# leonzheng2/Safe-Exploration-with-Simulator-in-RL-algorithms

Hardware: AMD Instinct MI355X
Metric: env-steps/sec (higher is better)
Workload: dtype f64; 1 GPU; ARS V2 iteration, 3-segment swimmer, 512 directions/GPU x 2 rollouts x H=1000 (BASELINE configs[2] per GPU); directions_total=512, directions_per_gpu=512, horizon=1000, segments=3, trajectory_capture=True, full_covariance=True, parallelism=directions sharded over 1 GPU(s), 1 all-gather/iteration, ranks_seen=1

## Files before the change

include/swimmer_hip.h:

```cpp
#ifndef SWIMMER_HIP_H
#define SWIMMER_HIP_H

#include <stdint.h>

#ifdef __cplusplus
extern "C" {
#endif

#define SW_ABI_VERSION 3
#define SW_MAX_SEGMENTS 8

#define SW_OK 0
#define SW_ERR_NULL 1
#define SW_ERR_SEGMENTS 2
#define SW_ERR_SIZE 3
#define SW_ERR_PARAM 4
#define SW_ERR_LAUNCH 5

#define SW_STATUS_OK 0
#define SW_STATUS_SINGULAR 1
#define SW_STATUS_NONFINITE 2
#define SW_STATUS_RANGE 4
#define SW_STATUS_PARAM 8

#define SW_FLAG_ROLLOUT_LANE 1
#define SW_FLAG_ROLLOUT_QUAD 2

#define SW_FLAG_CAPTURE_SPLIT 8
#define SW_FLAG_CAPTURE_PACKED_V1 16
#define SW_FLAG_CAPTURE_LEAN_V1 128

#define SW_FLAG_MODEL_TWIN 4

typedef struct sw_params {
    int32_t n;
    int32_t flags;
    double l_i;
    double m_i;
    double k;
    double h;
    double dir_x;
    double dir_y;
} sw_params;

int sw_abi_version(void);
// ... 229 lines not shown
```

safe-exploration-with-simulator-in-rl-algorithms_amd/_build.py:

```python
import os
import shutil
import subprocess
import tempfile
from concurrent.futures import ThreadPoolExecutor

_HERE = os.path.dirname(os.path.abspath(__file__))
CSRC = os.path.join(_HERE, "csrc")
LIB_PATH = os.environ.get("SWIMMER_HIP_LIB") or os.path.join(CSRC, "libswimmer_hip.so")
OBJ_DIR = LIB_PATH + ".obj"
SOURCES = ["swimmer_kernels.hip", "swimmer_abi.hip", "swimmer_cacla.hip", "swimmer_lqr.hip", "swimmer_cacla_safe.hip",
           "swimmer_cacla_ensemble.hip", "swimmer_rlglue_ars.hip", "swimmer_safe_ars_ensemble.hip", "direct_comm.cpp",
           "host_rng.cpp"]
FAMILIES = ["swimmer_rollout_row.hip", "swimmer_rollout_n3.hip", "swimmer_rollout_lane.hip",
            "swimmer_rollout_safe_multi.hip", "swimmer_step.hip", "swimmer_cov.hip", "swimmer_update.hip"]
HOST_ONLY = {"host_rng.cpp"}
HEADERS = ["rlglue_env.cpp", os.path.join("..", "..", "include", "rlglue_swimmer.h"),
           "swimmer_launch.h", "swimmer_cov.h", "swimmer_device.h", "swimmer_rollout_lane.inc",
           "swimmer_rollout_quad3.inc", "swimmer_rollout_oct3.inc", "swimmer_rollout_octp3.inc",
           "swimmer_rollout_row.inc", "swimmer_rollout_multi.inc", "swimmer_rollout_safe_oct3.inc",
           "swimmer_rollout_safe_lane.inc", "swimmer_rollout_safe_multi.inc", "swimmer_update.inc", "swimmer_quad3.h",
           "swimmer_oct3.h", "swimmer_row.h", "swimmer_row_fused.h", "swimmer_twin.h", "swimmer_cacla_learner.h",
           "swimmer_cacla_gated.h", os.path.join("..", "..", "include", "swimmer_hip.h")] + FAMILIES
HIPCC_FLAGS = ["-O3", "--offload-arch=gfx950", "-std=c++17", "-fPIC"] + os.environ.get("SWIMMER_HIPCC_EXTRA", "").split()
HOST_FLAGS = ["-O3", "-std=c++17", "-fPIC"]
LINK_LIBS = ["-ldl"]
LLVM = "/opt/rocm/lib/llvm/bin"


def _hipcc():
    exe = shutil.which("hipcc") or "/opt/rocm/bin/hipcc"
    if not os.path.exists(exe):
        raise RuntimeError("hipcc not found: the swimmer HIP library cannot be built")
    return exe
# ... 79 lines not shown
```

safe-exploration-with-simulator-in-rl-algorithms_amd/_lib.py:

```python
import ctypes
import os

import numpy as np
import torch

from . import _build

ABI_VERSION = 3
MAX_SEGMENTS = 8

ERR_NAMES = {0: "SW_OK", 1: "SW_ERR_NULL", 2: "SW_ERR_SEGMENTS", 3: "SW_ERR_SIZE",
             4: "SW_ERR_PARAM", 5: "SW_ERR_LAUNCH"}
STATUS_SINGULAR = 1
STATUS_NONFINITE = 2
STATUS_RANGE = 4
STATUS_PARAM = 8
FLAG_ROLLOUT_LANE = 1
FLAG_ROLLOUT_QUAD = 2
FLAG_MODEL_TWIN = 4
FLAG_CAPTURE_SPLIT = 8
FLAG_CAPTURE_PACKED_V1 = 16
FLAG_CAPTURE_LEAN_V1 = 128
COST_ABS_OBS = 0
COST_MAX_ABS_THETADOT = 1


class SwParams(ctypes.Structure):
    _fields_ = [("n", ctypes.c_int32), ("flags", ctypes.c_int32), ("l_i", ctypes.c_double),
                ("m_i", ctypes.c_double), ("k", ctypes.c_double), ("h", ctypes.c_double),
                ("dir_x", ctypes.c_double), ("dir_y", ctypes.c_double)]

    @classmethod
    def make(cls, n=3, l_i=1.0, m_i=1.0, k=10.0, h=1e-3, direction=(1.0, 0.0), flags=0):
        return cls(int(n), int(flags), float(l_i), float(m_i), float(k), float(h),
                   float(direction[0]), float(direction[1]))

    @property
    def d(self):
        return 2 * self.n + 2

    @property
    def m(self):
        return self.n - 1


class SwimmerHipError(RuntimeError):
    pass


def kernel_flags(name):
    try:
        return {"auto": 0, "lane": FLAG_ROLLOUT_LANE, "quad": FLAG_ROLLOUT_QUAD, "split": FLAG_CAPTURE_SPLIT,
                "packed_v1": FLAG_CAPTURE_PACKED_V1, "lean_v1": FLAG_CAPTURE_LEAN_V1}[name]
    except KeyError:
        raise SwimmerHipError("rollout kernel must be 'auto', 'lane', 'quad', 'split', 'packed_v1' or 'lean_v1', "
                              f"not {name!r}")


_lib = None

_PROTOTYPES = {
    "sw_abi_version": (ctypes.c_int, []),
    "sw_max_segments": (ctypes.c_int, []),
    "sw_strerror": (ctypes.c_char_p, [ctypes.c_int]),
    "sw_moments_blocks": (ctypes.c_int64, [ctypes.c_int64]),
    "sw_reset_f64": (ctypes.c_int, [ctypes.c_void_p, ctypes.c_int64, ctypes.c_void_p,
                                    ctypes.c_void_p]),
    "sw_step_f64": (ctypes.c_int, [ctypes.c_void_p, ctypes.c_int64] + [ctypes.c_void_p] * 6),
    "sw_step_residual_f64": (ctypes.c_int, [ctypes.c_void_p, ctypes.c_int64] + [ctypes.c_void_p] * 5),
    "sw_step_residual_blocks": (ctypes.c_int64, [ctypes.c_int64]),
    "sw_step_residual_pop_f64": (ctypes.c_int, [ctypes.c_void_p, ctypes.c_int64, ctypes.c_void_p, ctypes.c_int64]
# ... 208 lines not shown
```

safe-exploration-with-simulator-in-rl-algorithms_amd/csrc/swimmer_launch.h:

```cpp
#pragma once
#include <hip/hip_runtime.h>
#include <math.h>
#include <stdint.h>
#include <climits>
#include <cstdlib>
#include <type_traits>
#include <utility>

#include "../../include/swimmer_hip.h"
#include "swimmer_device.h"
#include "swimmer_twin.h"

#define SW_PIN_LOOP(PAD) asm volatile(".p2align 6\n\t.fill %0, 4, 0xbf800000" ::"n"(PAD))
#ifndef SW_OCT_UNROLL
#define SW_OCT_UNROLL 8
#endif
#ifdef SW_OCT_LOOP_PAD
constexpr int oct_loop_pad(bool, bool) { return SW_OCT_LOOP_PAD; }
#else
constexpr int oct_loop_pad(bool traj, bool mom) { return traj ? (mom ? 5 : 6) : (mom ? 6 : 2); }
#endif
#ifndef SW_OCTP_LOOP_PAD
#define SW_OCTP_LOOP_PAD 4
#endif
constexpr int oct_packed_loop_pad() { return SW_OCTP_LOOP_PAD; }
#ifndef SW_OCTL_LOOP_PAD
#define SW_OCTL_LOOP_PAD 2
#endif
constexpr int oct_lean_loop_pad() { return SW_OCTL_LOOP_PAD; }
#ifndef SW_OCTS_LOOP_PAD
#define SW_OCTS_LOOP_PAD 2
#endif
constexpr int oct_next_e_loop_pad() { return SW_OCTS_LOOP_PAD; }
#ifndef SW_OCTS_TRIP16
#define SW_OCTS_TRIP16 1
#endif
#ifndef SW_QUAD_LOOP_PAD
#define SW_QUAD_LOOP_PAD 0
#endif
#ifdef SW_ROW_LOOP_PAD
constexpr int row_loop_pad(int, bool, bool) { return SW_ROW_LOOP_PAD; }
#else
constexpr int row_loop_pad(int n, bool traj, bool mom)
{
    if (n == 6 && !(traj && mom)) return traj ? 6 : 4;
    return n == 4 ? 5 : n == 5 ? 0 : n == 6 ? 5 : n == 7 ? 6 : 1;
}
#endif

#ifdef SW_MULTI_LOOP_PAD
// ... 77 lines not shown
    return sw::consts_of(p->n, p->l_i, p->m_i, p->k, p->h, p->dir_x, p->dir_y);
}

sw::TwinConsts make_twin_consts(const sw_params *p)
{
    return sw::TwinConsts{p->l_i, p->m_i, p->k, p->h, p->dir_x, p->dir_y};
}

inline bool is_twin(const sw_params *p) { return (p->flags & SW_FLAG_MODEL_TWIN) != 0; }

int validate_params(const sw_params *p)
{
    if (!p) return SW_ERR_NULL;
    if (p->n < 2 || p->n > SW_MAX_SEGMENTS) return SW_ERR_SEGMENTS;
    if (p->flags & ~(SW_FLAG_ROLLOUT_LANE | SW_FLAG_ROLLOUT_QUAD | SW_FLAG_MODEL_TWIN | SW_FLAG_CAPTURE_SPLIT |
                     SW_FLAG_CAPTURE_PACKED_V1 | SW_FLAG_CAPTURE_LEAN_V1))
        return SW_ERR_PARAM;
    if ((p->flags & SW_FLAG_CAPTURE_SPLIT) && (p->flags & SW_FLAG_CAPTURE_PACKED_V1)) return SW_ERR_PARAM;
    if ((p->flags & SW_FLAG_CAPTURE_LEAN_V1) && (p->flags & (SW_FLAG_CAPTURE_SPLIT | SW_FLAG_CAPTURE_PACKED_V1)))
        return SW_ERR_PARAM;
    if (!(p->l_i > 0.0) || !(p->m_i > 0.0) || !isfinite(p->l_i) || !isfinite(p->m_i) ||
        !isfinite(p->k) || !isfinite(p->h) || !isfinite(p->dir_x) || !isfinite(p->dir_y))
        return SW_ERR_PARAM;
    return SW_OK;
}

int check_params(const sw_params *p)
{
    (void)hipGetLastError();
    return validate_params(p);
}

int launch_status()
{
// ... 263 lines not shown
```

safe-exploration-with-simulator-in-rl-algorithms_amd/csrc/swimmer_rollout_n3.hip:

```cpp
#include "swimmer_cov.h"
#include "swimmer_quad3.h"
#include "swimmer_oct3.h"

namespace {

template <bool ARS, bool TRAJ, bool MOM>
__global__ void __launch_bounds__(kRollBlock)
rollout_quad3_kernel(sw::Consts C, int64_t n_roll, int32_t H, const double *__restrict__ policies,
                     const double *__restrict__ deltas, int64_t dir_begin, double nu,
                     const double *__restrict__ mean, const double *__restrict__ inv_std,
                     const double *__restrict__ state0, double *__restrict__ returns,
                     double *__restrict__ traj, double *__restrict__ final_state,
                     double *__restrict__ moments, int32_t *__restrict__ status, SideJob side)
{
#define SW_GATE_BODY 0
#include "swimmer_rollout_quad3.inc"
#undef SW_GATE_BODY
}

__global__ void __launch_bounds__(kRollBlock)
ars_gate_quad3_kernel(sw::Consts C, int64_t n_roll, int32_t H, const double *__restrict__ policies,
                      const double *__restrict__ deltas, int64_t dir_begin, double nu,
                      const double *__restrict__ mean, const double *__restrict__ inv_std, double gate_thr,
                      int32_t *__restrict__ admit, double *__restrict__ returns, int32_t *__restrict__ status,
// ... 39 lines not shown
#include "swimmer_rollout_oct3.inc"
#undef SW_GATE_BODY
}

template <bool ARS>
__global__ void __launch_bounds__(kOctBlock)
rollout_octp3_kernel(sw::Consts C, int64_t n_roll, int32_t H, const double *__restrict__ policies,
                     const double *__restrict__ deltas, int64_t dir_begin, double nu,
                     const double *__restrict__ mean, const double *__restrict__ inv_std,
                     const double *__restrict__ state0, double *__restrict__ returns,
                     double *__restrict__ traj, double *__restrict__ final_state,
                     double *__restrict__ moments, int32_t *__restrict__ status, SideJob side)
{
#define SW_OCTP_LEAN 0
#define SW_OCTP_NEXT_E 0
#include "swimmer_rollout_octp3.inc"
#undef SW_OCTP_NEXT_E
#undef SW_OCTP_LEAN
}

template <bool ARS>
__global__ void __launch_bounds__(kOctBlock)
rollout_octl3_kernel(sw::Consts C, int64_t n_roll, int32_t H, const double *__restrict__ policies,
                     const double *__restrict__ deltas, int64_t dir_begin, double nu,
                     const double *__restrict__ mean, const double *__restrict__ inv_std,
                     const double *__restrict__ state0, double *__restrict__ returns,
                     double *__restrict__ traj, double *__restrict__ final_state,
                     double *__restrict__ moments, int32_t *__restrict__ status, SideJob side)
{
#define SW_OCTP_LEAN 1
#define SW_OCTP_NEXT_E 0
#include "swimmer_rollout_octp3.inc"
#undef SW_OCTP_NEXT_E
#undef SW_OCTP_LEAN
}

template <bool ARS>
__global__ void __launch_bounds__(kOctBlock)
rollout_octs3_kernel(sw::Consts C, int64_t n_roll, int32_t H, const double *__restrict__ policies,
                     const double *__restrict__ deltas, int64_t dir_begin, double nu,
                     const double *__restrict__ mean, const double *__restrict__ inv_std,
                     const double *__restrict__ state0, double *__restrict__ returns,
                     double *__restrict__ traj, double *__restrict__ final_state,
                     double *__restrict__ moments, int32_t *__restrict__ status, SideJob side)
{
#define SW_OCTP_LEAN 1
#define SW_OCTP_NEXT_E 1
#include "swimmer_rollout_octp3.inc"
#undef SW_OCTP_NEXT_E
#undef SW_OCTP_LEAN
}

#define SW_MULTI_N 3
template <bool MOM>
__global__ void __launch_bounds__(kRollBlock)
ars_multi_quad3_kernel(sw::Consts C, int64_t n_roll, int32_t H, sw_launch::MultiArgs all, double nu, SideJob side)
{
    constexpr bool ARS = true, TRAJ = false;
#include "swimmer_rollout_multi.inc"
#define SW_GATE_BODY 0
#include "swimmer_rollout_quad3.inc"
#undef SW_GATE_BODY
}
// ... 105 lines not shown
                         double sim_thresh, double real_thresh, double *__restrict__ returns,
                         double *__restrict__ traj, int32_t *__restrict__ first_refused,
                         int32_t *__restrict__ violations, int32_t *__restrict__ status)
{
#define SW_SAFE_MULTI 0
#include "swimmer_rollout_safe_oct3.inc"
#undef SW_SAFE_MULTI
}

using namespace sw_launch;

int launch_oct3(const sw_params *p, const RolloutPlan &plan, bool ars, int64_t n_roll, int32_t H, const RolloutArgs &a,
                hipStream_t stream, const SideWork *side)
{
    if (a.traj && a.moments && !(p->flags & SW_FLAG_CAPTURE_SPLIT)) {
        with_bools([&](auto ARS, auto V1, auto LEAN_V1) {
            if constexpr (V1.value)
                launch_segment_per_lane(rollout_octp3_kernel<ARS.value>, p, plan, n_roll, H, a, stream, side);
            else if constexpr (LEAN_V1.value)
                launch_segment_per_lane(rollout_octl3_kernel<ARS.value>, p, plan, n_roll, H, a, stream, side);
            else
                launch_segment_per_lane(rollout_octs3_kernel<ARS.value>, p, plan, n_roll, H, a, stream, side);
        }, ars, (p->flags & SW_FLAG_CAPTURE_PACKED_V1) != 0, (p->flags & SW_FLAG_CAPTURE_LEAN_V1) != 0);
        return launch_status();
    }
    with_bools([&](auto ARS, auto TRAJ, auto MOM) {
        launch_segment_per_lane(rollout_oct3_kernel<ARS.value, TRAJ.value, MOM.value>, p, plan, n_roll, H, a, stream,
                                side);
    }, ars, a.traj != nullptr, a.moments != nullptr);
    return launch_status();
}

int launch_quad3(const sw_params *p, const RolloutPlan &plan, bool ars, int64_t n_roll, int32_t H,
                 const RolloutArgs &a, hipStream_t stream, const SideWork *side)
{
    with_bools([&](auto ARS, auto TRAJ, auto MOM) {
        launch_segment_per_lane(rollout_quad3_kernel<ARS.value, TRAJ.value, MOM.value>, p, plan, n_roll, H, a, stream,
// ... 118 lines not shown
```

safe-exploration-with-simulator-in-rl-algorithms_amd/csrc/swimmer_rollout_octp3.inc:

```
#ifndef SW_OCTP_LEAN
#error "define SW_OCTP_LEAN as 0 or 1 before including swimmer_rollout_octp3.inc"
#endif
#ifndef SW_OCTP_NEXT_E
#error "define SW_OCTP_NEXT_E as 0 or 1 before including swimmer_rollout_octp3.inc"
#endif
#if SW_OCTP_NEXT_E && !SW_OCTP_LEAN
#error "SW_OCTP_NEXT_E is a variant of the lean mode"
#endif
    side_flag(side);
    if (blockIdx.x >= side.first_cov_block) {
        side_cov_tile<8, kOctBlock>(side);
        return;
    }
    __builtin_amdgcn_s_setprio(3);
    constexpr int D = 8, M = 2;
    const int tid = threadIdx.x, lane = tid & (kWave - 1), wave = tid / kWave;
    const int q = lane & 3;
    const int seg = (q == 3) ? 0 : q;
    const bool cosine = (lane & 8) != 0;
    const int64_t r_raw = (int64_t)blockIdx.x * kMomGroup + wave * 8 + (lane >> 4) * 2 + ((lane >> 2) & 1);
    const bool valid = r_raw < n_roll;
    const int64_t r = valid ? r_raw : n_roll - 1;
    const sw::OctLane O = sw::oct3_lane(C, seg, cosine);
    const int cth = 2 + 2 * seg, cthd = 3 + 2 * seg;
// ... 100 lines not shown
        Gx = sw::oct3_geometry(A);
        det = sw::oct3_dynamics(C, O, Gc, Pu, Pv, thd, w1, w2, tq);
#endif
        const double Z = sw::octp3_pack(__builtin_fma(A.kd, sw::kPio2Hi, A.r), thd, Pu, lane3);
        const double X = Z - shift;
        m1 += X;
        m2 = __builtin_fma(X, X, m2);
        store_cell(Z);
#if !SW_OCTP_LEAN
        soff += slab;
#endif
        w1 = sw::dpp_f64<sw::kDppNext1>(thd);
        w2 = sw::dpp_f64<sw::kDppNext2>(thd);
        Pv = sw::dpp_row_f64<sw::kDppRowRor8>(Pu);
    };
    int32_t t = 0;
#if SW_OCTP_NEXT_E
    SW_PIN_LOOP(oct_next_e_loop_pad());
#else
    SW_PIN_LOOP(SW_OCTP_LEAN ? oct_lean_loop_pad() : oct_packed_loop_pad());
#endif
#if SW_OCTP_NEXT_E && SW_OCTS_TRIP16
    for (; t + 16 <= H; t += 16) {
        SW_OCTP_STEP_AT(0);   one_step(G, Gn);
        SW_OCTP_STEP_AT(k1);  one_step(Gn, G);
        SW_OCTP_STEP_AT(k2);  one_step(G, Gn);
        SW_OCTP_STEP_AT(k3);  one_step(Gn, G);
        SW_OCTP_STEP_AT(k4);  one_step(G, Gn);
        SW_OCTP_STEP_AT(k5);  one_step(Gn, G);
        SW_OCTP_STEP_AT(k6);  one_step(G, Gn);
        SW_OCTP_STEP_AT(k7);  one_step(Gn, G);
        SW_OCTP_STEP_AT(k8);  one_step(G, Gn);
        SW_OCTP_STEP_AT(k9);  one_step(Gn, G);
        SW_OCTP_STEP_AT(k10); one_step(G, Gn);
        SW_OCTP_STEP_AT(k11); one_step(Gn, G);
        SW_OCTP_STEP_AT(k12); one_step(G, Gn);
        SW_OCTP_STEP_AT(k13); one_step(Gn, G);
        SW_OCTP_STEP_AT(k14); one_step(G, Gn);
        SW_OCTP_STEP_AT(k15); one_step(Gn, G);
        SW_OCTP_TRIP_END(bump16);
    }
#endif
    for (; t + 8 <= H; t += 8) {
        SW_OCTP_STEP_AT(0);  one_step(G, Gn);
        SW_OCTP_STEP_AT(k1); one_step(Gn, G);
        SW_OCTP_STEP_AT(k2); one_step(G, Gn);
        SW_OCTP_STEP_AT(k3); one_step(Gn, G);
        SW_OCTP_STEP_AT(k4); one_step(G, Gn);
        SW_OCTP_STEP_AT(k5); one_step(Gn, G);
        SW_OCTP_STEP_AT(k6); one_step(G, Gn);
        SW_OCTP_STEP_AT(k7); one_step(Gn, G);
        SW_OCTP_TRIP_END(bump8);
    }
    for (; t + 4 <= H; t += 4) {
        SW_OCTP_STEP_AT(0);  one_step(G, Gn);
        SW_OCTP_STEP_AT(k1); one_step(Gn, G);
        SW_OCTP_STEP_AT(k2); one_step(G, Gn);
        SW_OCTP_STEP_AT(k3); one_step(Gn, G);
        SW_OCTP_TRIP_END(bump4);
    }
    for (; t + 2 <= H; t += 2) {
        SW_OCTP_STEP_AT(0);  one_step(G, Gn);
        SW_OCTP_STEP_AT(k1); one_step(Gn, G);
        SW_OCTP_TRIP_END(bump2);
    }
    SW_OCTP_STEP_AT(0);
    if (t < H) one_step(G, Gn);
#undef SW_OCTP_STEP_AT
#undef SW_OCTP_TRIP_END
    if (H > 0) th = __builtin_fma(A.kd, sw::kPio2Hi, A.r);
    thmax = fmax(thmax, fabs(th));

    int code = ((det > 0.0) ? 0 : SW_STATUS_SINGULAR) |
               ((isfinite(th) && isfinite(thd) && isfinite(Pu) && isfinite(Pv)) ? 0 : SW_STATUS_NONFINITE) |
               ((thmax < sw::kAngleLimit) ? 0 : SW_STATUS_RANGE);
    code |= __builtin_amdgcn_mov_dpp(code, sw::kDppNext1, 0xf, 0xf, true) |
            __builtin_amdgcn_mov_dpp(code, sw::kDppNext2, 0xf, 0xf, true);
    code |= __builtin_amdgcn_mov_dpp(code, sw::kDppRowRor8, 0xf, 0xf, true);
    const double sg_other = sw::dpp_row_f64<sw::kDppRowRor8>(m1);
    if (valid && !cosine && lane3) {
        const double total = __builtin_fma(C.dirx, m1, C.diry * sg_other);
        returns[r] = (code & SW_STATUS_RANGE) ? __builtin_nan("") : total;
// ... 37 lines not shown
```

Before: 5.000 billion env-steps/s.

## Add hand-scheduled two-step fused rollout kernel as default trajectory-capture path

New measurement: 4.623 billion env-steps/s. 0.925x the previous value.

```diff
diff --git a/include/swimmer_hip.h b/include/swimmer_hip.h
--- a/include/swimmer_hip.h
+++ b/include/swimmer_hip.h
@@ -29,6 +29,7 @@
 #define SW_FLAG_CAPTURE_SPLIT 8
 #define SW_FLAG_CAPTURE_PACKED_V1 16
 #define SW_FLAG_CAPTURE_LEAN_V1 128
+#define SW_FLAG_CAPTURE_NEXT_E_V1 512
 
 #define SW_FLAG_MODEL_TWIN 4
 
diff --git a/safe-exploration-with-simulator-in-rl-algorithms_amd/_build.py b/safe-exploration-with-simulator-in-rl-algorithms_amd/_build.py
--- a/safe-exploration-with-simulator-in-rl-algorithms_amd/_build.py
+++ b/safe-exploration-with-simulator-in-rl-algorithms_amd/_build.py
@@ -16,7 +16,7 @@
 HOST_ONLY = {"host_rng.cpp"}
 HEADERS = ["rlglue_env.cpp", os.path.join("..", "..", "include", "rlglue_swimmer.h"),
            "swimmer_launch.h", "swimmer_cov.h", "swimmer_device.h", "swimmer_rollout_lane.inc",
-           "swimmer_rollout_quad3.inc", "swimmer_rollout_oct3.inc", "swimmer_rollout_octp3.inc",
+           "swimmer_rollout_quad3.inc", "swimmer_rollout_oct3.inc", "swimmer_rollout_octp3.inc", "swimmer_rollout_octf3_pair.inc",
            "swimmer_rollout_row.inc", "swimmer_rollout_multi.inc", "swimmer_rollout_safe_oct3.inc",
            "swimmer_rollout_safe_lane.inc", "swimmer_rollout_safe_multi.inc", "swimmer_update.inc", "swimmer_quad3.h",
            "swimmer_oct3.h", "swimmer_row.h", "swimmer_row_fused.h", "swimmer_twin.h", "swimmer_cacla_learner.h",
diff --git a/safe-exploration-with-simulator-in-rl-algorithms_amd/_lib.py b/safe-exploration-with-simulator-in-rl-algorithms_amd/_lib.py
--- a/safe-exploration-with-simulator-in-rl-algorithms_amd/_lib.py
+++ b/safe-exploration-with-simulator-in-rl-algorithms_amd/_lib.py
@@ -21,6 +21,7 @@
 FLAG_CAPTURE_SPLIT = 8
 FLAG_CAPTURE_PACKED_V1 = 16
 FLAG_CAPTURE_LEAN_V1 = 128
+FLAG_CAPTURE_NEXT_E_V1 = 512
 COST_ABS_OBS = 0
 COST_MAX_ABS_THETADOT = 1
 
@@ -51,10 +52,11 @@
 def kernel_flags(name):
     try:
         return {"auto": 0, "lane": FLAG_ROLLOUT_LANE, "quad": FLAG_ROLLOUT_QUAD, "split": FLAG_CAPTURE_SPLIT,
-                "packed_v1": FLAG_CAPTURE_PACKED_V1, "lean_v1": FLAG_CAPTURE_LEAN_V1}[name]
+                "packed_v1": FLAG_CAPTURE_PACKED_V1, "lean_v1": FLAG_CAPTURE_LEAN_V1,
+                "next_e_v1": FLAG_CAPTURE_NEXT_E_V1}[name]
     except KeyError:
-        raise SwimmerHipError("rollout kernel must be 'auto', 'lane', 'quad', 'split', 'packed_v1' or 'lean_v1', "
-                              f"not {name!r}")
+        raise SwimmerHipError("rollout kernel must be 'auto', 'lane', 'quad', 'split', 'packed_v1', 'lean_v1' or "
+                              f"'next_e_v1', not {name!r}")
 
 
 _lib = None
diff --git a/safe-exploration-with-simulator-in-rl-algorithms_amd/csrc/swimmer_launch.h b/safe-exploration-with-simulator-in-rl-algorithms_amd/csrc/swimmer_launch.h
--- a/safe-exploration-with-simulator-in-rl-algorithms_amd/csrc/swimmer_launch.h
+++ b/safe-exploration-with-simulator-in-rl-algorithms_amd/csrc/swimmer_launch.h
@@ -34,6 +34,13 @@
 constexpr int oct_next_e_loop_pad() { return SW_OCTS_LOOP_PAD; }
 #ifndef SW_OCTS_TRIP16
 #define SW_OCTS_TRIP16 1
+#endif
+#ifndef SW_OCTF_LOOP_PAD
+#define SW_OCTF_LOOP_PAD 2
+#endif
+constexpr int oct_layout_loop_pad() { return SW_OCTF_LOOP_PAD; }
+#ifndef SW_OCTF_PROMOTE
+#define SW_OCTF_PROMOTE 0
 #endif
 #ifndef SW_QUAD_LOOP_PAD
 #define SW_QUAD_LOOP_PAD 0
@@ -141,10 +148,13 @@
     if (!p) return SW_ERR_NULL;
     if (p->n < 2 || p->n > SW_MAX_SEGMENTS) return SW_ERR_SEGMENTS;
     if (p->flags & ~(SW_FLAG_ROLLOUT_LANE | SW_FLAG_ROLLOUT_QUAD | SW_FLAG_MODEL_TWIN | SW_FLAG_CAPTURE_SPLIT |
-                     SW_FLAG_CAPTURE_PACKED_V1 | SW_FLAG_CAPTURE_LEAN_V1))
+                     SW_FLAG_CAPTURE_PACKED_V1 | SW_FLAG_CAPTURE_LEAN_V1 | SW_FLAG_CAPTURE_NEXT_E_V1))
         return SW_ERR_PARAM;
     if ((p->flags & SW_FLAG_CAPTURE_SPLIT) && (p->flags & SW_FLAG_CAPTURE_PACKED_V1)) return SW_ERR_PARAM;
     if ((p->flags & SW_FLAG_CAPTURE_LEAN_V1) && (p->flags & (SW_FLAG_CAPTURE_SPLIT | SW_FLAG_CAPTURE_PACKED_V1)))
+        return SW_ERR_PARAM;
+    if ((p->flags & SW_FLAG_CAPTURE_NEXT_E_V1) &&
+        (p->flags & (SW_FLAG_CAPTURE_SPLIT | SW_FLAG_CAPTURE_PACKED_V1 | SW_FLAG_CAPTURE_LEAN_V1)))
         return SW_ERR_PARAM;
     if (!(p->l_i > 0.0) || !(p->m_i > 0.0) || !isfinite(p->l_i) || !isfinite(p->m_i) ||
         !isfinite(p->k) || !isfinite(p->h) || !isfinite(p->dir_x) || !isfinite(p->dir_y))
diff --git a/safe-exploration-with-simulator-in-rl-algorithms_amd/csrc/swimmer_rollout_n3.hip b/safe-exploration-with-simulator-in-rl-algorithms_amd/csrc/swimmer_rollout_n3.hip
--- a/safe-exploration-with-simulator-in-rl-algorithms_amd/csrc/swimmer_rollout_n3.hip
+++ b/safe-exploration-with-simulator-in-rl-algorithms_amd/csrc/swimmer_rollout_n3.hip
@@ -77,7 +77,9 @@
 {
 #define SW_OCTP_LEAN 0
 #define SW_OCTP_NEXT_E 0
+#define SW_OCTP_LAYOUT 0
 #include "swimmer_rollout_octp3.inc"
+#undef SW_OCTP_LAYOUT
 #undef SW_OCTP_NEXT_E
 #undef SW_OCTP_LEAN
 }
@@ -93,7 +95,9 @@
 {
 #define SW_OCTP_LEAN 1
 #define SW_OCTP_NEXT_E 0
+#define SW_OCTP_LAYOUT 0
 #include "swimmer_rollout_octp3.inc"
+#undef SW_OCTP_LAYOUT
 #undef SW_OCTP_NEXT_E
 #undef SW_OCTP_LEAN
 }
@@ -109,7 +113,27 @@
 {
 #define SW_OCTP_LEAN 1
 #define SW_OCTP_NEXT_E 1
+#define SW_OCTP_LAYOUT 0
 #include "swimmer_rollout_octp3.inc"
+#undef SW_OCTP_LAYOUT
+#undef SW_OCTP_NEXT_E
+#undef SW_OCTP_LEAN
+}
+
+template <bool ARS>
+__global__ void __launch_bounds__(kOctBlock)
+rollout_octf3_kernel(sw::Consts C, int64_t n_roll, int32_t H, const double *__restrict__ policies,
+                     const double *__restrict__ deltas, int64_t dir_begin, double nu,
+                     const double *__restrict__ mean, const double *__restrict__ inv_std,
+                     const double *__restrict__ state0, double *__restrict__ returns,
+                     double *__restrict__ traj, double *__restrict__ final_state,
+                     double *__restrict__ moments, int32_t *__restrict__ status, SideJob side)
+{
+#define SW_OCTP_LEAN 1
+#define SW_OCTP_NEXT_E 1
+#define SW_OCTP_LAYOUT 1
+#include "swimmer_rollout_octp3.inc"
+#undef SW_OCTP_LAYOUT
 #undef SW_OCTP_NEXT_E
 #undef SW_OCTP_LEAN
 }
@@ -245,13 +269,19 @@
                 hipStream_t stream, const SideWork *side)
 {
     if (a.traj && a.moments && !(p->flags & SW_FLAG_CAPTURE_SPLIT)) {
+        if (p->flags & SW_FLAG_CAPTURE_NEXT_E_V1) {
+            with_bools([&](auto ARS) {
+                launch_segment_per_lane(rollout_octs3_kernel<ARS.value>, p, plan, n_roll, H, a, stream, side);
+            }, ars);
+            return launch_status();
+        }
         with_bools([&](auto ARS, auto V1, auto LEAN_V1) {
             if constexpr (V1.value)
                 launch_segment_per_lane(rollout_octp3_kernel<ARS.value>, p, plan, n_roll, H, a, stream, side);
             else if constexpr (LEAN_V1.value)
                 launch_segment_per_lane(rollout_octl3_kernel<ARS.value>, p, plan, n_roll, H, a, stream, side);
             else
-                launch_segment_per_lane(rollout_octs3_kernel<ARS.value>, p, plan, n_roll, H, a, stream, side);
+                launch_segment_per_lane(rollout_octf3_kernel<ARS.value>, p, plan, n_roll, H, a, stream, side);
         }, ars, (p->flags & SW_FLAG_CAPTURE_PACKED_V1) != 0, (p->flags & SW_FLAG_CAPTURE_LEAN_V1) != 0);
         return launch_status();
     }
diff --git a/safe-exploration-with-simulator-in-rl-algorithms_amd/csrc/swimmer_rollout_octf3_pair.inc b/safe-exploration-with-simulator-in-rl-algorithms_amd/csrc/swimmer_rollout_octf3_pair.inc
--- /dev/null
+++ b/safe-exploration-with-simulator-in-rl-algorithms_amd/csrc/swimmer_rollout_octf3_pair.inc
@@ -0,0 +1,203 @@
+    double Pu_a, Pu_b, Pv_a, Pv_b, Th_a, Th_b, X_a, X_b, Xr_a, Xr_b, Xz_a, Xz_b, Z_a, Z_b, a1c_a, a1c_b, a2c_a, a2c_b, a_a, a_b, ad2_a, ad2_b, b_a, b_b, bd1_a, bd1_b, c00_a, c00_b, c01_a, c01_b, c02_a, c02_b, cent_a, cent_b, det_a, det_b, e_a, e_b, fric_a, fric_b, g_a, g_b, gn1_a, gn1_b, gn2_a, gn2_b, k1c_a, k1c_b, k2c_a, k2c_b, m1_a, m1_b, m2_a, m2_b, npu_a, npu_b, num_a, num_b, p_a, p_b, r0_a, r0_b, r1_a, r1_b, r2_a, r2_b, rc0_a, rc0_b, rc_a, rc_b, rce_a, rce_b, su_a, su_b, tdd_a, tdd_b, thd_a, thd_b, thf_a, thf_b, tq_a, tq_b, uv1_a, uv1_b, uv2_a, uv2_b, vv1_a, vv1_b, vv2_a, vv2_b, w1_a, w1_b, w2_a, w2_b, ww1_a, ww1_b, ww2_a, ww2_b, xcc1_a, xcc1_b, xcc2_a, xcc2_b, xf1_a, xf1_b, xf2_a, xf2_b, xu1_a, xu1_b, xu2_a, xu2_b, xu_a, xu_b, xv1_a, xv1_b, xv2_a, xv2_b, xv_a, xv_b, z_a, z_b;
+    int zlo_a, zhi_a, zlo_b, zhi_b;
+    npu_a = -Pu * G.u; asm volatile("" : "+v"(npu_a)); __builtin_amdgcn_sched_barrier(0);
+    tq_a = __builtin_fma(VPu, Pu, Th); asm volatile("" : "+v"(tq_a)); __builtin_amdgcn_sched_barrier(0);
+    k1c_a = O.kvw1 * G.cc1; asm volatile("" : "+v"(k1c_a)); __builtin_amdgcn_sched_barrier(0);
+    g_a = __builtin_fma(Pv, G.v, npu_a); asm volatile("" : "+v"(g_a)); __builtin_amdgcn_sched_barrier(0);
+    A.r = __builtin_fma(C.h, thd, A.r); asm volatile("" : "+v"(A.r)); __builtin_amdgcn_sched_barrier(0);
+    tq_a = __builtin_fma(VPv, Pv, tq_a); asm volatile("" : "+v"(tq_a)); __builtin_amdgcn_sched_barrier(0);
+    g_a = __builtin_fma(O.kvw0, thd, g_a); asm volatile("" : "+v"(g_a)); __builtin_amdgcn_sched_barrier(0);
+    k2c_a = O.kvw2 * G.cc2; asm volatile("" : "+v"(k2c_a)); __builtin_amdgcn_sched_barrier(0);
+    const unsigned long long outside_a = sw::oct3_range_test_vcc(A.r); __builtin_amdgcn_sched_barrier(0);
+    g_a = __builtin_fma(k1c_a, w1, g_a); asm volatile("" : "+v"(g_a)); __builtin_amdgcn_sched_barrier(0);
+    tq_a = __builtin_fma(V[3], thd, tq_a); asm volatile("" : "+v"(tq_a)); __builtin_amdgcn_sched_barrier(0);
+    sw::oct3_keep_reduced_vcc(A, thmax, magic, designation, outside_a); __builtin_amdgcn_sched_barrier(0);
+    g_a = __builtin_fma(k2c_a, w2, g_a); asm volatile("" : "+v"(g_a)); __builtin_amdgcn_sched_barrier(0);
+    tq_a = __builtin_fma(V[5], w1, tq_a); asm volatile("" : "+v"(tq_a)); __builtin_amdgcn_sched_barrier(0);
+    z_a = A.r * A.r; asm volatile("" : "+v"(z_a)); __builtin_amdgcn_sched_barrier(0);
+    ww1_a = w1 * w1; asm volatile("" : "+v"(ww1_a)); __builtin_amdgcn_sched_barrier(0);
+    tq_a = __builtin_fma(V[7], w2, tq_a); asm volatile("" : "+v"(tq_a)); __builtin_amdgcn_sched_barrier(0);
+    p_a = sw::fma3(A.k[0], z_a, A.k[1]); __builtin_amdgcn_sched_barrier(0);
+    gn1_a = sw::dpp_f64<sw::kDppNext1>(g_a); asm volatile("" : "+v"(gn1_a)); __builtin_amdgcn_sched_barrier(0);
+    ww1_a = O.kt1 * ww1_a; asm volatile("" : "+v"(ww1_a)); __builtin_amdgcn_sched_barrier(0);
+    ww2_a = w2 * w2; asm volatile("" : "+v"(ww2_a)); __builtin_amdgcn_sched_barrier(0);
+    fric_a = O.ka0 * g_a; asm volatile("" : "+v"(fric_a)); __builtin_amdgcn_sched_barrier(0);
+    a1c_a = O.ka1 * G.cc1; asm volatile("" : "+v"(a1c_a)); __builtin_amdgcn_sched_barrier(0);
+    a_a = O.t1 * G.cc1; asm volatile("" : "+v"(a_a)); __builtin_amdgcn_sched_barrier(0);
+    b_a = O.t2 * G.cc2; asm volatile("" : "+v"(b_a)); __builtin_amdgcn_sched_barrier(0);
+    p_a = sw::fma3(p_a, z_a, A.k[2]); __builtin_amdgcn_sched_barrier(0);
+    gn2_a = sw::dpp_f64<sw::kDppNext2>(g_a); asm volatile("" : "+v"(gn2_a)); __builtin_amdgcn_sched_barrier(0);
+    cent_a = __builtin_fma(ww1_a, G.f1, tq_a); asm volatile("" : "+v"(cent_a)); __builtin_amdgcn_sched_barrier(0);
+    ww2_a = O.kt2 * ww2_a; asm volatile("" : "+v"(ww2_a)); __builtin_amdgcn_sched_barrier(0);
+    SW_OCTF_FMA(0, fric_a, a1c_a, gn1_a, fric_a); __builtin_amdgcn_sched_barrier(0);
+    a2c_a = O.ka2 * G.cc2; asm volatile("" : "+v"(a2c_a)); __builtin_amdgcn_sched_barrier(0);
+    e_a = sw::dpp_f64<sw::kDppNext1>(a_a); asm volatile("" : "+v"(e_a)); __builtin_amdgcn_sched_barrier(0);
+    bd1_a = -b_a * O.d1; asm volatile("" : "+v"(bd1_a)); __builtin_amdgcn_sched_barrier(0);
+    p_a = sw::fma3(p_a, z_a, A.k[3]); __builtin_amdgcn_sched_barrier(0);
+    cent_a = __builtin_fma(ww2_a, G.f2, cent_a); asm volatile("" : "+v"(cent_a)); __builtin_amdgcn_sched_barrier(0);
+    fric_a = __builtin_fma(a2c_a, gn2_a, fric_a); asm volatile("" : "+v"(fric_a)); __builtin_amdgcn_sched_barrier(0);
+    ad2_a = -a_a * O.d2; asm volatile("" : "+v"(ad2_a)); __builtin_amdgcn_sched_barrier(0);
+    c02_a = __builtin_fma(a_a, e_a, bd1_a); asm volatile("" : "+v"(c02_a)); __builtin_amdgcn_sched_barrier(0);
+    p_a = sw::fma3(p_a, z_a, A.k[4]); __builtin_amdgcn_sched_barrier(0);
+    r0_a = __builtin_fma(-C.six_k_m, fric_a, cent_a); asm volatile("" : "+v"(r0_a)); __builtin_amdgcn_sched_barrier(0);
+    SW_OCTF_FMA(1, c01_a, b_a, e_a, ad2_a); __builtin_amdgcn_sched_barrier(0);
+    det_a = b_a * c02_a; asm volatile("" : "+v"(det_a)); __builtin_amdgcn_sched_barrier(0);
+    p_a = sw::fma3(p_a, z_a, A.k[5]); __builtin_amdgcn_sched_barrier(0);
+    X_a = __builtin_fma(A.selS, A.r, A.selC); asm volatile("" : "+v"(X_a)); __builtin_amdgcn_sched_barrier(0);
+    r0_a = __builtin_fma(C.kl_m, thd, r0_a); asm volatile("" : "+v"(r0_a)); __builtin_amdgcn_sched_barrier(0);
+    c00_a = __builtin_fma(-e_a, e_a, O.d12); asm volatile("" : "+v"(c00_a)); __builtin_amdgcn_sched_barrier(0);
+    det_a = __builtin_fma(a_a, c01_a, det_a); asm volatile("" : "+v"(det_a)); __builtin_amdgcn_sched_barrier(0);
+    p_a = sw::fma3(p_a, z_a, A.k[6]); __builtin_amdgcn_sched_barrier(0);
+    Xz_a = X_a * z_a; asm volatile("" : "+v"(Xz_a)); __builtin_amdgcn_sched_barrier(0);
+    su_a = g_a * G.u; asm volatile("" : "+v"(su_a)); __builtin_amdgcn_sched_barrier(0);
+    r2_a = sw::dpp_f64<sw::kDppNext2>(r0_a); asm volatile("" : "+v"(r2_a)); __builtin_amdgcn_sched_barrier(0);
+    det_a = __builtin_fma(O.d0, c00_a, det_a); asm volatile("" : "+v"(det_a)); __builtin_amdgcn_sched_barrier(0);
+    xu_a = __builtin_fma(Xz_a, p_a, X_a); asm volatile("" : "+v"(xu_a)); __builtin_amdgcn_sched_barrier(0);
+    SW_OCTF_FMA(2, su_a, gn1_a, G.u1, su_a); __builtin_amdgcn_sched_barrier(0);
+    r1_a = sw::dpp_f64<sw::kDppNext1>(r0_a); asm volatile("" : "+v"(r1_a)); __builtin_amdgcn_sched_barrier(0);
+    num_a = c02_a * r2_a; asm volatile("" : "+v"(num_a)); __builtin_amdgcn_sched_barrier(0);
+    rc0_a = __builtin_amdgcn_rcp(det_a); asm volatile("" : "+v"(rc0_a)); __builtin_amdgcn_sched_barrier(0);
+    xv_a = sw::dpp_row_f64<sw::kDppRowRor8>(xu_a); asm volatile("" : "+v"(xv_a)); __builtin_amdgcn_sched_barrier(0);
+    su_a = __builtin_fma(gn2_a, G.u2, su_a); asm volatile("" : "+v"(su_a)); __builtin_amdgcn_sched_barrier(0);
+    num_a = __builtin_fma(c01_a, r1_a, num_a); asm volatile("" : "+v"(num_a)); __builtin_amdgcn_sched_barrier(0);
+    rce_a = __builtin_fma(-det_a, rc0_a, 1.0); asm volatile("" : "+v"(rce_a)); __builtin_amdgcn_sched_barrier(0);
+    Th_a = __builtin_fma(hV2, thd, Th); asm volatile("" : "+v"(Th_a)); __builtin_amdgcn_sched_barrier(0);
+    num_a = __builtin_fma(c00_a, r0_a, num_a); asm volatile("" : "+v"(num_a)); __builtin_amdgcn_sched_barrier(0);
+    rc_a = __builtin_fma(rc0_a, rce_a, rc0_a); asm volatile("" : "+v"(rc_a)); __builtin_amdgcn_sched_barrier(0);
+    Pu_a = __builtin_fma(C.h_kl_nm, su_a, Pu); asm volatile("" : "+v"(Pu_a)); __builtin_amdgcn_sched_barrier(0);
+    xv1_a = sw::dpp_f64<sw::kDppNext1>(xv_a); asm volatile("" : "+v"(xv1_a)); __builtin_amdgcn_sched_barrier(0);
+    SW_OCTF_FMA(3, Th_a, hV4, w1, Th_a); __builtin_amdgcn_sched_barrier(0);
+    tdd_a = num_a * rc_a; asm volatile("" : "+v"(tdd_a)); __builtin_amdgcn_sched_barrier(0);
+    xu1_a = sw::dpp_f64<sw::kDppNext1>(xu_a); asm volatile("" : "+v"(xu1_a)); __builtin_amdgcn_sched_barrier(0);
+    xv2_a = sw::dpp_f64<sw::kDppNext2>(xv_a); asm volatile("" : "+v"(xv2_a)); __builtin_amdgcn_sched_barrier(0);
+    vv1_a = xv_a * xv1_a; asm volatile("" : "+v"(vv1_a)); __builtin_amdgcn_sched_barrier(0);
+    Pv_a = sw::dpp_row_f64<sw::kDppRowRor8>(Pu_a); asm volatile("" : "+v"(Pv_a)); __builtin_amdgcn_sched_barrier(0);
+    npu_b = -Pu_a * xu_a; asm volatile("" : "+v"(npu_b)); __builtin_amdgcn_sched_barrier(0);
+    SW_OCTF_FMA(4, Th_a, hV6, w2, Th_a); __builtin_amdgcn_sched_barrier(0);
+    thd_a = __builtin_fma(C.h, tdd_a, thd); asm volatile("" : "+v"(thd_a)); __builtin_amdgcn_sched_barrier(0);
+    xu2_a = sw::dpp_f64<sw::kDppNext2>(xu_a); asm volatile("" : "+v"(xu2_a)); __builtin_amdgcn_sched_barrier(0);
+    SW_OCTF_FMA(5, xcc1_a, xu_a, xu1_a, vv1_a); __builtin_amdgcn_sched_barrier(0);
+    vv2_a = xv_a * xv2_a; asm volatile("" : "+v"(vv2_a)); __builtin_amdgcn_sched_barrier(0);
+    g_b = __builtin_fma(Pv_a, xv_a, npu_b); asm volatile("" : "+v"(g_b)); __builtin_amdgcn_sched_barrier(0);
+    tq_b = __builtin_fma(VPu, Pu_a, Th_a); asm volatile("" : "+v"(tq_b)); __builtin_amdgcn_sched_barrier(0);
+    SW_OCTF_FMA(6, xcc2_a, xu_a, xu2_a, vv2_a); __builtin_amdgcn_sched_barrier(0);
+    thf_a = __builtin_fma(A.kd, sw::kPio2Hi, A.r); asm volatile("" : "+v"(thf_a)); __builtin_amdgcn_sched_barrier(0);
+    w1_a = sw::dpp_f64<sw::kDppNext1>(thd_a); asm volatile("" : "+v"(w1_a)); __builtin_amdgcn_sched_barrier(0);
+    SW_OCTF_FMA(7, g_b, O.kvw0, thd_a, g_b); __builtin_amdgcn_sched_barrier(0);
+    k1c_b = O.kvw1 * xcc1_a; asm volatile("" : "+v"(k1c_b)); __builtin_amdgcn_sched_barrier(0);
+    A.r = __builtin_fma(C.h, thd_a, A.r); asm volatile("" : "+v"(A.r)); __builtin_amdgcn_sched_barrier(0);
+    SW_OCTF_FMA(8, tq_b, VPv, Pv_a, tq_b); __builtin_amdgcn_sched_barrier(0);
+    w2_a = sw::dpp_f64<sw::kDppNext2>(thd_a); asm volatile("" : "+v"(w2_a)); __builtin_amdgcn_sched_barrier(0);
+    SW_OCTF_FMA(9, g_b, k1c_b, w1_a, g_b); __builtin_amdgcn_sched_barrier(0);
+    k2c_b = O.kvw2 * xcc2_a; asm volatile("" : "+v"(k2c_b)); __builtin_amdgcn_sched_barrier(0);
+    const unsigned long long outside_b = sw::oct3_range_test_vcc(A.r); __builtin_amdgcn_sched_barrier(0);
+    tq_b = __builtin_fma(V[3], thd_a, tq_b); asm volatile("" : "+v"(tq_b)); __builtin_amdgcn_sched_barrier(0);
+    sw::oct3_keep_reduced_vcc(A, thmax, magic, designation, outside_b); __builtin_amdgcn_sched_barrier(0);
+    g_b = __builtin_fma(k2c_b, w2_a, g_b); asm volatile("" : "+v"(g_b)); __builtin_amdgcn_sched_barrier(0);
+    uv1_a = -xu_a * xv1_a; asm volatile("" : "+v"(uv1_a)); __builtin_amdgcn_sched_barrier(0);
+    SW_OCTF_FMA(10, tq_b, V[5], w1_a, tq_b); __builtin_amdgcn_sched_barrier(0);
+    z_b = A.r * A.r; asm volatile("" : "+v"(z_b)); __builtin_amdgcn_sched_barrier(0);
+    ww1_b = w1_a * w1_a; asm volatile("" : "+v"(ww1_b)); __builtin_amdgcn_sched_barrier(0);
+    SW_OCTF_FMA(11, xf1_a, xv_a, xu1_a, uv1_a); __builtin_amdgcn_sched_barrier(0);
+    uv2_a = -xu_a * xv2_a; asm volatile("" : "+v"(uv2_a)); __builtin_amdgcn_sched_barrier(0);
+    tq_b = __builtin_fma(V[7], w2_a, tq_b); asm volatile("" : "+v"(tq_b)); __builtin_amdgcn_sched_barrier(0);
+    p_b = sw::fma3(A.k[0], z_b, A.k[1]); __builtin_amdgcn_sched_barrier(0);
+    gn1_b = sw::dpp_f64<sw::kDppNext1>(g_b); asm volatile("" : "+v"(gn1_b)); __builtin_amdgcn_sched_barrier(0);
+    ww1_b = O.kt1 * ww1_b; asm volatile("" : "+v"(ww1_b)); __builtin_amdgcn_sched_barrier(0);
+    ww2_b = w2_a * w2_a; asm volatile("" : "+v"(ww2_b)); __builtin_amdgcn_sched_barrier(0);
+    fric_b = O.ka0 * g_b; asm volatile("" : "+v"(fric_b)); __builtin_amdgcn_sched_barrier(0);
+    a1c_b = O.ka1 * xcc1_a; asm volatile("" : "+v"(a1c_b)); __builtin_amdgcn_sched_barrier(0);
+    a_b = O.t1 * xcc1_a; asm volatile("" : "+v"(a_b)); __builtin_amdgcn_sched_barrier(0);
+    b_b = O.t2 * xcc2_a; asm volatile("" : "+v"(b_b)); __builtin_amdgcn_sched_barrier(0);
+    xf2_a = __builtin_fma(xv_a, xu2_a, uv2_a); asm volatile("" : "+v"(xf2_a)); __builtin_amdgcn_sched_barrier(0);
+    p_b = sw::fma3(p_b, z_b, A.k[2]); __builtin_amdgcn_sched_barrier(0);
+    gn2_b = sw::dpp_f64<sw::kDppNext2>(g_b); asm volatile("" : "+v"(gn2_b)); __builtin_amdgcn_sched_barrier(0);
+    cent_b = __builtin_fma(ww1_b, xf1_a, tq_b); asm volatile("" : "+v"(cent_b)); __builtin_amdgcn_sched_barrier(0);
+    ww2_b = O.kt2 * ww2_b; asm volatile("" : "+v"(ww2_b)); __builtin_amdgcn_sched_barrier(0);
+    SW_OCTF_FMA(12, fric_b, a1c_b, gn1_b, fric_b); __builtin_amdgcn_sched_barrier(0);
+    a2c_b = O.ka2 * xcc2_a; asm volatile("" : "+v"(a2c_b)); __builtin_amdgcn_sched_barrier(0);
+    e_b = sw::dpp_f64<sw::kDppNext1>(a_b); asm volatile("" : "+v"(e_b)); __builtin_amdgcn_sched_barrier(0);
+    bd1_b = -b_b * O.d1; asm volatile("" : "+v"(bd1_b)); __builtin_amdgcn_sched_barrier(0);
+    p_b = sw::fma3(p_b, z_b, A.k[3]); __builtin_amdgcn_sched_barrier(0);
+    cent_b = __builtin_fma(ww2_b, xf2_a, cent_b); asm volatile("" : "+v"(cent_b)); __builtin_amdgcn_sched_barrier(0);
+    fric_b = __builtin_fma(a2c_b, gn2_b, fric_b); asm volatile("" : "+v"(fric_b)); __builtin_amdgcn_sched_barrier(0);
+    ad2_b = -a_b * O.d2; asm volatile("" : "+v"(ad2_b)); __builtin_amdgcn_sched_barrier(0);
+    c02_b = __builtin_fma(a_b, e_b, bd1_b); asm volatile("" : "+v"(c02_b)); __builtin_amdgcn_sched_barrier(0);
+    p_b = sw::fma3(p_b, z_b, A.k[4]); __builtin_amdgcn_sched_barrier(0);
+    r0_b = __builtin_fma(-C.six_k_m, fric_b, cent_b); asm volatile("" : "+v"(r0_b)); __builtin_amdgcn_sched_barrier(0);
+    SW_OCTF_FMA(13, c01_b, b_b, e_b, ad2_b); __builtin_amdgcn_sched_barrier(0);
+    det_b = b_b * c02_b; asm volatile("" : "+v"(det_b)); __builtin_amdgcn_sched_barrier(0);
+    p_b = sw::fma3(p_b, z_b, A.k[5]); __builtin_amdgcn_sched_barrier(0);
+    X_b = __builtin_fma(A.selS, A.r, A.selC); asm volatile("" : "+v"(X_b)); __builtin_amdgcn_sched_barrier(0);
+    r0_b = __builtin_fma(C.kl_m, thd_a, r0_b); asm volatile("" : "+v"(r0_b)); __builtin_amdgcn_sched_barrier(0);
+    c00_b = __builtin_fma(-e_b, e_b, O.d12); asm volatile("" : "+v"(c00_b)); __builtin_amdgcn_sched_barrier(0);
+    det_b = __builtin_fma(a_b, c01_b, det_b); asm volatile("" : "+v"(det_b)); __builtin_amdgcn_sched_barrier(0);
+    p_b = sw::fma3(p_b, z_b, A.k[6]); __builtin_amdgcn_sched_barrier(0);
+    Xz_b = X_b * z_b; asm volatile("" : "+v"(Xz_b)); __builtin_amdgcn_sched_barrier(0);
+    su_b = g_b * xu_a; asm volatile("" : "+v"(su_b)); __builtin_amdgcn_sched_barrier(0);
+    r2_b = sw::dpp_f64<sw::kDppNext2>(r0_b); asm volatile("" : "+v"(r2_b)); __builtin_amdgcn_sched_barrier(0);
+    det_b = __builtin_fma(O.d0, c00_b, det_b); asm volatile("" : "+v"(det_b)); __builtin_amdgcn_sched_barrier(0);
+    xu_b = __builtin_fma(Xz_b, p_b, X_b); asm volatile("" : "+v"(xu_b)); __builtin_amdgcn_sched_barrier(0);
+    SW_OCTF_FMA(14, su_b, gn1_b, xu1_a, su_b); __builtin_amdgcn_sched_barrier(0);
+    r1_b = sw::dpp_f64<sw::kDppNext1>(r0_b); asm volatile("" : "+v"(r1_b)); __builtin_amdgcn_sched_barrier(0);
+    num_b = c02_b * r2_b; asm volatile("" : "+v"(num_b)); __builtin_amdgcn_sched_barrier(0);
+    rc0_b = __builtin_amdgcn_rcp(det_b); asm volatile("" : "+v"(rc0_b)); __builtin_amdgcn_sched_barrier(0);
+    xv_b = sw::dpp_row_f64<sw::kDppRowRor8>(xu_b); asm volatile("" : "+v"(xv_b)); __builtin_amdgcn_sched_barrier(0);
+    su_b = __builtin_fma(gn2_b, xu2_a, su_b); asm volatile("" : "+v"(su_b)); __builtin_amdgcn_sched_barrier(0);
+    num_b = __builtin_fma(c01_b, r1_b, num_b); asm volatile("" : "+v"(num_b)); __builtin_amdgcn_sched_barrier(0);
+    rce_b = __builtin_fma(-det_b, rc0_b, 1.0); asm volatile("" : "+v"(rce_b)); __builtin_amdgcn_sched_barrier(0);
+    Th_b = __builtin_fma(hV2, thd_a, Th_a); asm volatile("" : "+v"(Th_b)); __builtin_amdgcn_sched_barrier(0);
+    num_b = __builtin_fma(c00_b, r0_b, num_b); asm volatile("" : "+v"(num_b)); __builtin_amdgcn_sched_barrier(0);
+    rc_b = __builtin_fma(rc0_b, rce_b, rc0_b); asm volatile("" : "+v"(rc_b)); __builtin_amdgcn_sched_barrier(0);
+    Pu_b = __builtin_fma(C.h_kl_nm, su_b, Pu_a); asm volatile("" : "+v"(Pu_b)); __builtin_amdgcn_sched_barrier(0);
+    xv1_b = sw::dpp_f64<sw::kDppNext1>(xv_b); asm volatile("" : "+v"(xv1_b)); __builtin_amdgcn_sched_barrier(0);
+    SW_OCTF_FMA(15, Th_b, hV4, w1_a, Th_b); __builtin_amdgcn_sched_barrier(0);
+    tdd_b = num_b * rc_b; asm volatile("" : "+v"(tdd_b)); __builtin_amdgcn_sched_barrier(0);
+    xu1_b = sw::dpp_f64<sw::kDppNext1>(xu_b); asm volatile("" : "+v"(xu1_b)); __builtin_amdgcn_sched_barrier(0);
+    xv2_b = sw::dpp_f64<sw::kDppNext2>(xv_b); asm volatile("" : "+v"(xv2_b)); __builtin_amdgcn_sched_barrier(0);
+    vv1_b = xv_b * xv1_b; asm volatile("" : "+v"(vv1_b)); __builtin_amdgcn_sched_barrier(0);
+    Pv_b = sw::dpp_row_f64<sw::kDppRowRor8>(Pu_b); asm volatile("" : "+v"(Pv_b)); __builtin_amdgcn_sched_barrier(0);
+    SW_OCTF_FMA(16, Th_b, hV6, w2_a, Th_b); __builtin_amdgcn_sched_barrier(0);
+    thd_b = __builtin_fma(C.h, tdd_b, thd_a); asm volatile("" : "+v"(thd_b)); __builtin_amdgcn_sched_barrier(0);
+    xu2_b = sw::dpp_f64<sw::kDppNext2>(xu_b); asm volatile("" : "+v"(xu2_b)); __builtin_amdgcn_sched_barrier(0);
+    SW_OCTF_FMA(17, xcc1_b, xu_b, xu1_b, vv1_b); __builtin_amdgcn_sched_barrier(0);
+    vv2_b = xv_b * xv2_b; asm volatile("" : "+v"(vv2_b)); __builtin_amdgcn_sched_barrier(0);
+    thf_b = __builtin_fma(A.kd, sw::kPio2Hi, A.r); asm volatile("" : "+v"(thf_b)); __builtin_amdgcn_sched_barrier(0);
+    w1_b = sw::dpp_f64<sw::kDppNext1>(thd_b); asm volatile("" : "+v"(w1_b)); __builtin_amdgcn_sched_barrier(0);
+    SW_OCTF_FMA(18, xcc2_b, xu_b, xu2_b, vv2_b); __builtin_amdgcn_sched_barrier(0);
+    w2_b = sw::dpp_f64<sw::kDppNext2>(thd_b); asm volatile("" : "+v"(w2_b)); __builtin_amdgcn_sched_barrier(0);
+    uv1_b = -xu_b * xv1_b; asm volatile("" : "+v"(uv1_b)); __builtin_amdgcn_sched_barrier(0);
+    uv2_b = -xu_b * xv2_b; asm volatile("" : "+v"(uv2_b)); __builtin_amdgcn_sched_barrier(0);
+    zlo_a = __builtin_amdgcn_update_dpp(__double2loint(thf_a), __double2loint(thd_a), sw::kDppRowRor8, 0xf, 0xc, false); zhi_a = __builtin_amdgcn_update_dpp(__double2hiint(thf_a), __double2hiint(thd_a), sw::kDppRowRor8, 0xf, 0xc, false); asm volatile("" : "+v"(zlo_a)); asm volatile("" : "+v"(zhi_a)); __builtin_amdgcn_sched_barrier(0);
+    xf1_b = __builtin_fma(xv_b, xu1_b, uv1_b); asm volatile("" : "+v"(xf1_b)); __builtin_amdgcn_sched_barrier(0);
+    xf2_b = __builtin_fma(xv_b, xu2_b, uv2_b); asm volatile("" : "+v"(xf2_b)); __builtin_amdgcn_sched_barrier(0);
+    zlo_b = __builtin_amdgcn_update_dpp(__double2loint(thf_b), __double2loint(thd_b), sw::kDppRowRor8, 0xf, 0xc, false); zhi_b = __builtin_amdgcn_update_dpp(__double2hiint(thf_b), __double2hiint(thd_b), sw::kDppRowRor8, 0xf, 0xc, false); asm volatile("" : "+v"(zlo_b)); asm volatile("" : "+v"(zhi_b)); __builtin_amdgcn_sched_barrier(0);
+    Z_a = lane3 ? Pu_a : __hiloint2double(zhi_a, zlo_a); asm volatile("" : "+v"(Z_a)); __builtin_amdgcn_sched_barrier(0);
+    Z_b = lane3 ? Pu_b : __hiloint2double(zhi_b, zlo_b); asm volatile("" : "+v"(Z_b)); __builtin_amdgcn_sched_barrier(0);
+    Xr_a = Z_a - shift; asm volatile("" : "+v"(Xr_a)); __builtin_amdgcn_sched_barrier(0);
+    soff = KA; store_cell(Z_a); __builtin_amdgcn_sched_barrier(0);
+    Xr_b = Z_b - shift; asm volatile("" : "+v"(Xr_b)); __builtin_amdgcn_sched_barrier(0);
+    m1_a = m1 + Xr_a; asm volatile("" : "+v"(m1_a)); __builtin_amdgcn_sched_barrier(0);
+    SW_OCTF_FMA(19, m2_a, Xr_a, Xr_a, m2); __builtin_amdgcn_sched_barrier(0);
+    soff = KB; store_cell(Z_b); __builtin_amdgcn_sched_barrier(0);
+    m1_b = m1_a + Xr_b; asm volatile("" : "+v"(m1_b)); __builtin_amdgcn_sched_barrier(0);
+    SW_OCTF_FMA(20, m2_b, Xr_b, Xr_b, m2_a); __builtin_amdgcn_sched_barrier(0);
+    thd = thd_b;
+    Pu = Pu_b;
+    Pv = Pv_b;
+    w1 = w1_b;
+    w2 = w2_b;
+    Th = Th_b;
+    m1 = m1_b;
+    m2 = m2_b;
+    G.u = xu_b;
+    G.v = xv_b;
+    G.u1 = xu1_b;
+    G.v1 = xv1_b;
+    G.u2 = xu2_b;
+    G.v2 = xv2_b;
+    G.cc1 = xcc1_b;
+    G.cc2 = xcc2_b;
+    G.f1 = xf1_b;
+    G.f2 = xf2_b;
+    det = det_b;
diff --git a/safe-exploration-with-simulator-in-rl-algorithms_amd/csrc/swimmer_rollout_octp3.inc b/safe-exploration-with-simulator-in-rl-algorithms_amd/csrc/swimmer_rollout_octp3.inc
--- a/safe-exploration-with-simulator-in-rl-algorithms_amd/csrc/swimmer_rollout_octp3.inc
+++ b/safe-exploration-with-simulator-in-rl-algorithms_amd/csrc/swimmer_rollout_octp3.inc
@@ -6,6 +6,12 @@
 #endif
 #if SW_OCTP_NEXT_E && !SW_OCTP_LEAN
 #error "SW_OCTP_NEXT_E is a variant of the lean mode"
+#endif
+#ifndef SW_OCTP_LAYOUT
+#error "define SW_OCTP_LAYOUT as 0 or 1 before including swimmer_rollout_octp3.inc"
+#endif
+#if SW_OCTP_LAYOUT && !SW_OCTP_NEXT_E
+#error "SW_OCTP_LAYOUT is a variant of the mode with the neighbour's entry"
 #endif
     side_flag(side);
     if (blockIdx.x >= side.first_cov_block) {
@@ -138,58 +144,62 @@
         w2 = sw::dpp_f64<sw::kDppNext2>(thd);
         Pv = sw::dpp_row_f64<sw::kDppRowRor8>(Pu);
     };
+#if SW_OCTP_LAYOUT
+#define SW_OCTF_FMA(k, dst, a, b, c)                  \
+    if constexpr ((k) < SW_OCTF_PROMOTE) {            \
+        dst = sw::fma3(a, b, c);                      \
+    } else {                                          \
+        dst = __builtin_fma(a, b, c);                 \
+        asm volatile("" : "+v"(dst));                 \
+    }
+    auto two_steps = [&](uint32_t KA, uint32_t KB) {
+#include "swimmer_rollout_octf3_pair.inc"
+    };
+#undef SW_OCTF_FMA
+#define SW_OCTP_PAIR(KA, KB) two_steps(KA, KB)
+#else
+#define SW_OCTP_PAIR(KA, KB) SW_OCTP_STEP_AT(KA); one_step(G, Gn); SW_OCTP_STEP_AT(KB); one_step(Gn, G)
+#endif
     int32_t t = 0;
-#if SW_OCTP_NEXT_E
+#if SW_OCTP_LAYOUT
+    SW_PIN_LOOP(oct_layout_loop_pad());
+#elif SW_OCTP_NEXT_E
     SW_PIN_LOOP(oct_next_e_loop_pad());
 #else
     SW_PIN_LOOP(SW_OCTP_LEAN ? oct_lean_loop_pad() : oct_packed_loop_pad());
 #endif
 #if SW_OCTP_NEXT_E && SW_OCTS_TRIP16
     for (; t + 16 <= H; t += 16) {
-        SW_OCTP_STEP_AT(0);   one_step(G, Gn);
-        SW_OCTP_STEP_AT(k1);  one_step(Gn, G);
-        SW_OCTP_STEP_AT(k2);  one_step(G, Gn);
-        SW_OCTP_STEP_AT(k3);  one_step(Gn, G);
-        SW_OCTP_STEP_AT(k4);  one_step(G, Gn);
-        SW_OCTP_STEP_AT(k5);  one_step(Gn, G);
-        SW_OCTP_STEP_AT(k6);  one_step(G, Gn);
-        SW_OCTP_STEP_AT(k7);  one_step(Gn, G);
-        SW_OCTP_STEP_AT(k8);  one_step(G, Gn);
-        SW_OCTP_STEP_AT(k9);  one_step(Gn, G);
-        SW_OCTP_STEP_AT(k10); one_step(G, Gn);
-        SW_OCTP_STEP_AT(k11); one_step(Gn, G);
-        SW_OCTP_STEP_AT(k12); one_step(G, Gn);
-        SW_OCTP_STEP_AT(k13); one_step(Gn, G);
-        SW_OCTP_STEP_AT(k14); one_step(G, Gn);
-        SW_OCTP_STEP_AT(k15); one_step(Gn, G);
+        SW_OCTP_PAIR(0, k1);
+        SW_OCTP_PAIR(k2, k3);
+        SW_OCTP_PAIR(k4, k5);
+        SW_OCTP_PAIR(k6, k7);
+        SW_OCTP_PAIR(k8, k9);
+        SW_OCTP_PAIR(k10, k11);
+        SW_OCTP_PAIR(k12, k13);
+        SW_OCTP_PAIR(k14, k15);
         SW_OCTP_TRIP_END(bump16);
     }
 #endif
     for (; t + 8 <= H; t += 8) {
-        SW_OCTP_STEP_AT(0);  one_step(G, Gn);
-        SW_OCTP_STEP_AT(k1); one_step(Gn, G);
-        SW_OCTP_STEP_AT(k2); one_step(G, Gn);
-        SW_OCTP_STEP_AT(k3); one_step(Gn, G);
-        SW_OCTP_STEP_AT(k4); one_step(G, Gn);
-        SW_OCTP_STEP_AT(k5); one_step(Gn, G);
-        SW_OCTP_STEP_AT(k6); one_step(G, Gn);
-        SW_OCTP_STEP_AT(k7); one_step(Gn, G);
+        SW_OCTP_PAIR(0, k1);
+        SW_OCTP_PAIR(k2, k3);
+        SW_OCTP_PAIR(k4, k5);
+        SW_OCTP_PAIR(k6, k7);
         SW_OCTP_TRIP_END(bump8);
     }
     for (; t + 4 <= H; t += 4) {
-        SW_OCTP_STEP_AT(0);  one_step(G, Gn);
-        SW_OCTP_STEP_AT(k1); one_step(Gn, G);
-        SW_OCTP_STEP_AT(k2); one_step(G, Gn);
-        SW_OCTP_STEP_AT(k3); one_step(Gn, G);
+        SW_OCTP_PAIR(0, k1);
+        SW_OCTP_PAIR(k2, k3);
         SW_OCTP_TRIP_END(bump4);
     }
     for (; t + 2 <= H; t += 2) {
-        SW_OCTP_STEP_AT(0);  one_step(G, Gn);
-        SW_OCTP_STEP_AT(k1); one_step(Gn, G);
+        SW_OCTP_PAIR(0, k1);
         SW_OCTP_TRIP_END(bump2);
     }
     SW_OCTP_STEP_AT(0);
     if (t < H) one_step(G, Gn);
+#undef SW_OCTP_PAIR
 #undef SW_OCTP_STEP_AT
 #undef SW_OCTP_TRIP_END
     if (H > 0) th = __builtin_fma(A.kd, sw::kPio2Hi, A.r);
```
